# Alxkov/PSA-simulation-ODE-RK-MVP-Dispersion

Hardware: AMD Instinct MI355X
Metric: RK4 field-point updates/sec (sweep_pts x n_fields x n_zsteps / wall_s) (higher is better)
Workload: dtype f64

## Files before the change

psa-simulation-ode-rk-mvp-dispersion_amd/csrc/psa_rk4_kernel.inc.h:

```cpp
#pragma once
#include <type_traits>

#include "psa_internal.h"
#include "psa_rk4.h"

namespace psa {

__device__ __forceinline__ double fma_(double a, double b, double c) { return __builtin_fma(a, b, c); }
__device__ __forceinline__ float fma_(float a, float b, float c) { return __builtin_fmaf(a, b, c); }
typedef float f32x2 __attribute__((ext_vector_type(2)));
__device__ __forceinline__ f32x2 fma_(f32x2 a, f32x2 b, f32x2 c) { return __builtin_elementwise_fma(a, b, c); }

template <typename T> struct PairOf;
template <> struct PairOf<double> { typedef double type __attribute__((ext_vector_type(2))); };
template <> struct PairOf<float> { typedef float type __attribute__((ext_vector_type(2))); };

#ifndef PSA_TRAJ_F64_MOD
#define PSA_TRAJ_F64_MOD " nt"
#endif
__device__ __forceinline__ void store_pair_nt(const void *sbase, const unsigned voff, const PairOf<double>::type v) {
    asm volatile("global_store_dwordx4 %0, %1, %2" PSA_TRAJ_F64_MOD "\n\ts_nop 0\n\ts_nop 0" : : "v"(voff), "v"(v), "s"(sbase) : "memory");
}
__device__ __forceinline__ void store_pair_nt(const void *sbase, const unsigned voff, const PairOf<float>::type v) {
    asm volatile("global_store_dwordx2 %0, %1, %2 nt" : : "v"(voff), "v"(v), "s"(sbase) : "memory");
}
typedef float f32x4 __attribute__((ext_vector_type(4)));
__device__ __forceinline__ void store_quad_nt(const void *sbase, const unsigned voff, const f32x4 v) {
    asm volatile("global_store_dwordx4 %0, %1, %2 nt\n\ts_nop 0\n\ts_nop 0" : : "v"(voff), "v"(v), "s"(sbase) : "memory");
}

template <typename T> struct Phase;
template <> struct Phase<double> {
    static constexpr int RESYNC = 64;
    static __device__ __forceinline__ void eval(double ph, double &c, double &s) { sincos(ph, &s, &c); }
};
#ifndef PSA_F32_RESYNC
#define PSA_F32_RESYNC 16
#endif
template <> struct Phase<float> {
    static constexpr int RESYNC = PSA_F32_RESYNC;
    static __device__ __forceinline__ void eval(double ph, float &c, float &s) {
        const double r = ph - 6.283185307179586 * rint(ph * 0.15915494309189535);
        sincosf((float)r, &s, &c);
    }
};

template <typename T, int NW, bool FUSED, bool LOSS = true, bool CROSS = false, bool REALE = false>
__device__ __forceinline__ void yaman_stage(const T (&a)[2 * NW], const T (&base)[2 * NW],
                                            const T (&Er)[(NW - 2) / 2], const T (&Ei)[(NW - 2) / 2], const T g,
                                            const T tg, const T ha, T (&out)[2 * NW]) {
    static_assert(!REALE || (CROSS && NW == 4), "the real phase factor exists for the crosswise 4-wave stage");
    constexpr int NP = (NW - 2) / 2;
    T p[NW];
#pragma unroll
    for (int j = 0; j < NW; ++j) p[j] = fma_(a[2 * j], a[2 * j], a[2 * j + 1] * a[2 * j + 1]);
    T s = (p[0] + p[1]) + (p[2] + p[3]);
    if constexpr (NW == 6) s += (p[4] + p[5]);
    const T gs = tg * s;
    T gj[NW];
#pragma unroll
    for (int j = 0; j < NW; ++j) gj[j] = fma_(-g, p[j], gs);

    auto link = [&](const T gsig, const T v, const int c) -> T {
        if constexpr (LOSS) return fma_(gsig, v, FUSED ? fma_(ha, a[c], base[c]) : ha * a[c]);
        else return FUSED ? fma_(gsig, v, base[c]) : gsig * v;
    };

    const T x1 = a[0], y1 = a[1], x2 = a[2], y2 = a[3];
    if constexpr (CROSS && NW == 4) {
        const T x3 = a[4], y3 = a[5], x4 = a[6], y4 = a[7];
        const T b23r = fma_(x2, x3, y2 * y3), b23i = fma_(x2, y3, -(y2 * x3));
        const T b14r = fma_(x1, x4, y1 * y4), b14i = fma_(x1, y4, -(y1 * x4));
        const T h23r = REALE ? Er[0] * b23r : fma_(Er[0], b23r, -(Ei[0] * b23i));
        const T h23i = REALE ? Er[0] * b23i : fma_(Er[0], b23i, Ei[0] * b23r);
        const T h14r = REALE ? Er[0] * b14r : fma_(Er[0], b14r, -(Ei[0] * b14i));
        const T h14i = REALE ? Er[0] * b14i : fma_(Er[0], b14i, Ei[0] * b14r);
        out[0] = fma_(-y4, h23r, fma_(-x4, h23i, link(-gj[0], y1, 0)));
        out[1] = fma_(x4, h23r, fma_(-y4, h23i, link(gj[0], x1, 1)));
        out[2] = fma_(-y3, h14r, fma_(-x3, h14i, link(-gj[1], y2, 2)));
        out[3] = fma_(x3, h14r, fma_(-y3, h14i, link(gj[1], x2, 3)));
        out[4] = fma_(-y2, h14r, fma_(x2, h14i, link(-gj[2], y3, 4)));
        out[5] = fma_(x2, h14r, fma_(y2, h14i, link(gj[2], x3, 5)));
        out[6] = fma_(-y1, h23r, fma_(x1, h23i, link(-gj[3], y4, 6)));
        out[7] = fma_(x1, h23r, fma_(y1, h23i, link(gj[3], x4, 7)));
        return;
    }
    const T q12r = fma_(x1, x2, -(y1 * y2)), q12i = fma_(x1, y2, y1 * x2);

    T Fpr = T{}, Fpi = T{};
#pragma unroll
    for (int pr = 0; pr < NP; ++pr) {
        const int cs = 4 + 4 * pr;
        const T xs = a[cs], ys = a[cs + 1], xi = a[cs + 2], yi = a[cs + 3];
        const T qr = fma_(xs, xi, -(ys * yi)), qi = fma_(xs, yi, ys * xi);
        if (pr == 0) {
            Fpr = fma_(Er[pr], qr, -(Ei[pr] * qi));
            Fpi = fma_(Er[pr], qi, Ei[pr] * qr);
        } else {
            Fpr = fma_(Er[pr], qr, fma_(-Ei[pr], qi, Fpr));
            Fpi = fma_(Er[pr], qi, fma_(Ei[pr], qr, Fpi));
        }
        const T Fsr = fma_(Er[pr], q12r, Ei[pr] * q12i);
        const T Fsi = fma_(Er[pr], q12i, -(Ei[pr] * q12r));
        const T gS = gj[2 + 2 * pr], gI = gj[3 + 2 * pr];
        out[cs] = fma_(yi, Fsr, fma_(-xi, Fsi, link(-gS, ys, cs)));
        out[cs + 1] = fma_(xi, Fsr, fma_(yi, Fsi, link(gS, xs, cs + 1)));
        out[cs + 2] = fma_(ys, Fsr, fma_(-xs, Fsi, link(-gI, yi, cs + 2)));
        out[cs + 3] = fma_(xs, Fsr, fma_(ys, Fsi, link(gI, xi, cs + 3)));
    }
    out[0] = fma_(y2, Fpr, fma_(-x2, Fpi, link(-gj[0], y1, 0)));
    out[1] = fma_(x2, Fpr, fma_(y2, Fpi, link(gj[0], x1, 1)));
    out[2] = fma_(y1, Fpr, fma_(-x1, Fpi, link(-gj[1], y2, 2)));
    out[3] = fma_(x1, Fpr, fma_(y1, Fpi, link(gj[1], x2, 3)));
}

template <typename T, bool LOSS = true, bool FUSED = true, bool REALE = false>
__device__ __forceinline__ void yaman_stage_mirrored(const T (&a)[4], const T (&base)[4], const T Er, const T Ei, const T g,
                                                     const T sg, const T ha, T (&out)[4]) {
    const T x1 = a[0], y1 = a[1], xs = a[2], ys = a[3];
    const T p0 = fma_(x1, x1, y1 * y1), p2 = fma_(xs, xs, ys * ys);
    const T gs = sg * (p0 + p2);
    const T g1 = fma_(-g, p0, gs), g3 = fma_(-g, p2, gs);
    auto link = [&](const T gsig, const T v, const int c) -> T {
        if constexpr (LOSS) return fma_(gsig, v, FUSED ? fma_(ha, a[c], base[c]) : ha * a[c]);
        else return FUSED ? fma_(gsig, v, base[c]) : gsig * v;
    };
    const T br = fma_(x1, xs, y1 * ys), bi = fma_(x1, ys, -(y1 * xs));
    const T hr = REALE ? Er * br : fma_(Er, br, -(Ei * bi));
    const T hi = REALE ? Er * bi : fma_(Er, bi, Ei * br);
    out[0] = fma_(-ys, hr, fma_(-xs, hi, link(-g1, y1, 0)));
    out[1] = fma_(xs, hr, fma_(-ys, hi, link(g1, x1, 1)));
    out[2] = fma_(-y1, hr, fma_(x1, hi, link(-g3, ys, 2)));
    out[3] = fma_(x1, hr, fma_(y1, hi, link(g3, xs, 3)));
}

template <typename T, int NW, bool LOSS = true>
__device__ __forceinline__ void yaman_rhs(const T (&a)[2 * NW], const T (&Er)[(NW - 2) / 2],
                                          const T (&Ei)[(NW - 2) / 2], const T g, const T tg, const T ha,
                                          T (&k)[2 * NW]) {
    yaman_stage<T, NW, false, LOSS, true>(a, a, Er, Ei, g, tg, ha, k);
}

template <typename T>
__device__ __forceinline__ void rotate(T &Er, T &Ei, const T rc, const T rs) {
    const T nr = fma_(Er, rc, -(Ei * rs));
    const T ni = fma_(Er, rs, Ei * rc);
    Er = nr;
    Ei = ni;
}

template <typename T, int NC>
__device__ __forceinline__ bool any_nonfinite(const T (&y)[NC]) {
    T t = T(0);
#pragma unroll
    for (int c = 0; c < NC; ++c) t = fma_(y[c], T(0), t);
    return t != t;
}

#ifndef PSA_SWEEP_KERNEL_ATTR
#define PSA_SWEEP_KERNEL_ATTR
#endif
template <typename T, int NW, int CHECK, bool TRAJ, int BLOCK, bool LDS, bool LOSS, bool WSUM, bool MIRROR>
__device__ __forceinline__ void sweep_point(const SweepArgs<T> &A, const long long idx, T (&y)[MIRROR ? NW : 2 * NW]) {
    static_assert(!MIRROR || (sizeof(T) == 8 && NW == 4 && !LDS), "the mirrored body exists for the fused float64 4-wave step");
    constexpr int NC = 2 * NW;
    constexpr int NS = MIRROR ? NW : NC;
    constexpr int NWS = NS / 2;
    constexpr int SIG = MIRROR ? 2 : 4;
    constexpr int NP = (NW - 2) / 2;
    constexpr int RESYNC = Phase<T>::RESYNC;
    auto at = [](const int c) { return MIRROR ? (((c >> 2) << 1) | (c & 1)) : c; };
    const long long N = A.n_points;

    const T g = A.gamma[idx * A.gamma_stride];
    const T tg = g + g;
    const T ha = T(-0.5) * A.alpha[idx * A.alpha_stride];
    double dbd[NP];
    dbd[0] = (double)A.dbeta[idx];
    if constexpr (NP == 2) dbd[1] = (double)A.dbeta2[idx];

    const double hd = A.z_max / (double)A.n_steps;
    const T h = (T)hd, hh = (T)(0.5 * hd), h6 = (T)(hd / 6.0);
    const T g_d = hh * g, tg_d = hh * tg, ha_d = hh * ha;
    const T g_h = h * g, tg_h = h * tg, ha_h = h * ha;
    const T third = T(1.0 / 3.0);
    constexpr bool FUSE = (sizeof(T) == 8) && !LDS;
    const T e_amp = FUSE ? tg_d : tg;
    constexpr bool FRAME = FUSE && NW == 4;

    T rc[NP], rs[NP], Er[NP], Ei[NP];
#pragma unroll
    for (int p = 0; p < NP; ++p) {
        Phase<T>::eval(dbd[p] * (0.5 * hd), rc[p], rs[p]);
        Er[p] = e_amp;
        Ei[p] = T(0);
    }
    const T ec = e_amp * rc[0], es = e_amp * rs[0];
    auto frame_seed = [&](const int step, T &fc, T &fs) {
        Phase<T>::eval(dbd[0] * (0.5 * fma_((double)step, hd, 0.5 * hd)), fc, fs);
    };
    auto frame_at = [&](const int step, T &fc, T &fs) {
        const int k = step % RESYNC;
        frame_seed(step - k, fc, fs);
#pragma nounroll
        for (int q = 0; q < k; ++q) rotate(fc, fs, rc[0], rs[0]);
    };
    auto leave_frame = [&](const T (&b)[NS], const T fc, const T fs, T (&a)[NS]) {
        const T ce = T(-0.5) * fma_(fs, fs, fma_(fc, fc, T(-1)));
        const T nc = fma_(fc, ce, fc), ns = fma_(fs, ce, fs);
#pragma unroll
        for (int c = 0; c < SIG; ++c) a[c] = b[c];
#pragma unroll
        for (int c = SIG; c < NS; c += 2) {
            a[c] = fma_(b[c], nc, b[c + 1] * ns);
            a[c + 1] = fma_(b[c + 1], nc, -(b[c] * ns));
        }
    };
    T Fc = T(1), Fs = T(0);

    T pe = fma_(y[SIG], y[SIG], y[SIG + 1] * y[SIG + 1]);
    T pm = pe;
    long long bad = -1;
    T pwm[WSUM ? NWS : 1];
    if constexpr (WSUM) {
#pragma unroll
        for (int j = 0; j < NWS; ++j) pwm[j] = fma_(y[2 * j], y[2 * j], y[2 * j + 1] * y[2 * j + 1]);
    }
    auto store_a_end = [&](const T (&a)[NS]) {
#pragma unroll
        for (int c = 0; c < NC; ++c) A.a_end[(long long)c * N + idx] = a[at(c)];
        if constexpr (WSUM) {
#pragma unroll
            for (int j = 0; j < NW; ++j) {
                const T xr = y[at(2 * j)], xi = y[at(2 * j + 1)];
                A.p_wave_end[(long long)j * N + idx] = fma_(xr, xr, xi * xi);
            }
        }
    };

    const int se = A.save_every;
    const int n_rows = A.n_steps / se;
    const int n_run = (CHECK != CHECK_NONE) ? A.n_steps : n_rows * se;

    using Pair = typename PairOf<T>::type;
    const long long LD = A.traj_ld;
    const unsigned lane_off = (unsigned)idx * (unsigned)sizeof(Pair);
    auto store_traj_row_of = [&](const int r, const T (&a)[NS]) {
        const char *rowb = reinterpret_cast<const char *>(A.traj) + (long long)r * NW * LD * (long long)sizeof(Pair);
#pragma unroll
        for (int j = 0; j < NW; ++j)
            store_pair_nt(rowb + (long long)j * LD * (long long)sizeof(Pair), lane_off, Pair{a[at(2 * j)], a[at(2 * j + 1)]});
    };
    auto store_traj_row = [&](const int r) {
        if constexpr (FRAME) {
            T a[NS];
            leave_frame(y, Fc, Fs, a);
            store_traj_row_of(r, a);
        } else {
            store_traj_row_of(r, y);
        }
    };
    auto store_a_end_at = [&](const int step) {
        if constexpr (FRAME) {
            T a[NS], fc = Fc, fs = Fs;
            if constexpr (!TRAJ) frame_at(step, fc, fs);
            leave_frame(y, fc, fs, a);
            store_a_end(a);
        } else {
            store_a_end(y);
        }
    };
    if constexpr (TRAJ) store_traj_row_of(0, y);
    if (n_rows == 0) store_a_end(y);
    if constexpr (FRAME) {
        frame_seed(0, Fc, Fs);
#pragma unroll
        for (int c = SIG; c < NS; c += 2) rotate(y[c], y[c + 1], Fc, Fs);
    }

    __shared__ T sm_store[LDS ? 5 * NC * BLOCK : 1];
    volatile T *sm_y = sm_store + threadIdx.x;
    volatile T *sm_k = sm_store + NC * BLOCK + threadIdx.x;
    if constexpr (LDS) {
#pragma unroll
        for (int c = 0; c < NC; ++c) sm_y[c * BLOCK] = y[c];
    }
    auto rk4_step_lds = [&](const int step_index) {
        if constexpr (LDS) {
            T k[NC], ys[NC];
            const T coef[3] = {hh, hh, h};
#pragma unroll
            for (int c = 0; c < NC; ++c) ys[c] = sm_y[c * BLOCK];
#pragma unroll
            for (int st = 0; st < 4; ++st) {
                yaman_rhs<T, NW>(ys, Er, Ei, g, tg, ha, k);
#pragma unroll
                for (int c = 0; c < NC; ++c) sm_k[(st * NC + c) * BLOCK] = k[c];
                if (st == 0 || st == 2) {
#pragma unroll
                    for (int p = 0; p < NP; ++p) rotate(Er[p], Ei[p], rc[p], rs[p]);
                }
                if (st < 3) {
#pragma unroll
                    for (int c = 0; c < NC; ++c) ys[c] = fma_(coef[st], (T)sm_k[(st * NC + c) * BLOCK], (T)sm_y[c * BLOCK]);
                }
            }
#pragma unroll
            for (int c = 0; c < NC; ++c) {
                const T k1 = sm_k[(0 * NC + c) * BLOCK], k2 = sm_k[(1 * NC + c) * BLOCK];
                const T k3 = sm_k[(2 * NC + c) * BLOCK], k4 = sm_k[(3 * NC + c) * BLOCK];
                y[c] = fma_(h6, fma_(T(2), k3, fma_(T(2), k2, k1)) + k4, (T)sm_y[c * BLOCK]);
                sm_y[c * BLOCK] = y[c];
            }
            if constexpr (CHECK == CHECK_EXACT) {
                if (bad < 0 && any_nonfinite<T, NC>(y)) bad = step_index;
            }
        }
    };

    auto stage = [&](auto reale, const T (&a)[NS], const T (&base)[NS], const T (&er)[NP], const T (&ei)[NP], const T g_c,
                     const T tg_c, const T ha_c, T (&out)[NS]) {
        constexpr bool RE = decltype(reale)::value;
        if constexpr (MIRROR) yaman_stage_mirrored<T, LOSS, true, RE>(a, base, er[0], ei[0], g_c, tg_c + tg_c, ha_c, out);
        else yaman_stage<T, NW, true, LOSS, true, RE>(a, base, er, ei, g_c, tg_c, ha_c, out);
    };
    constexpr std::false_type cplx{};
    constexpr std::true_type real{};
    auto rk4_step_on = [&](T (&y)[NS], T (&Er)[NP], T (&Ei)[NP]) {
        T Y2[NS], Y3[NS], Y4[NS], t[NS], D[NS];
        if constexpr (FRAME) {
            const T c1[NP] = {ec}, s1[NP] = {-es}, s4[NP] = {es}, e1[NP] = {tg_d}, e2[NP] = {tg_h};
            stage(cplx, y, y, c1, s1, g_d, tg_d, ha_d, Y2);
            stage(real, Y2, y, e1, e1, g_d, tg_d, ha_d, Y3);
            stage(real, Y3, y, e2, e2, g_h, tg_h, ha_h, Y4);
#pragma unroll
            for (int c = 0; c < NS; ++c) t[c] = fma_(T(2), Y3[c], fma_(T(-4), y[c], Y2[c])) + Y4[c];
            stage(cplx, Y4, t, c1, s4, g_d, tg_d, ha_d, D);
#pragma unroll
            for (int c = 0; c < NS; ++c) y[c] = fma_(D[c], third, y[c]);
#pragma unroll
            for (int c = SIG; c < NS; c += 2) rotate(y[c], y[c + 1], rc[0], rs[0]);
            return;
        }
        stage(cplx, y, y, Er, Ei, g_d, tg_d, ha_d, Y2);
#pragma unroll
        for (int p = 0; p < NP; ++p) rotate(Er[p], Ei[p], rc[p], rs[p]);
        stage(cplx, Y2, y, Er, Ei, g_d, tg_d, ha_d, Y3);
        T E2r[NP], E2i[NP];
#pragma unroll
        for (int p = 0; p < NP; ++p) {
            E2r[p] = Er[p] + Er[p];
            E2i[p] = Ei[p] + Ei[p];
        }
        stage(cplx, Y3, y, E2r, E2i, g_h, tg_h, ha_h, Y4);
#pragma unroll
        for (int c = 0; c < NS; ++c) t[c] = fma_(T(2), Y3[c], fma_(T(-4), y[c], Y2[c])) + Y4[c];
#pragma unroll
        for (int p = 0; p < NP; ++p) rotate(Er[p], Ei[p], rc[p], rs[p]);
        stage(cplx, Y4, t, Er, Ei, g_d, tg_d, ha_d, D);
#pragma unroll
        for (int c = 0; c < NS; ++c) y[c] = fma_(D[c], third, y[c]);
    };
    auto rk4_step_reg = [&](const int) {
        rk4_step_on(y, Er, Ei);
        if constexpr (FRAME && TRAJ) rotate(Fc, Fs, rc[0], rs[0]);
    };

    T y_lo[NS];
#pragma unroll
    for (int c = 0; c < NS; ++c) y_lo[c] = T{};
    auto rk4_step_classic = [&](const int step_index) {
        if constexpr (!FUSE) {
            T k[NC], ys[NC], acc[NC];
            yaman_rhs<T, NW, LOSS>(y, Er, Ei, g, tg, ha, k);
#pragma unroll
            for (int c = 0; c < NC; ++c) {
                acc[c] = k[c];
                ys[c] = fma_(hh, k[c], y[c]);
            }
#pragma unroll
            for (int p = 0; p < NP; ++p) rotate(Er[p], Ei[p], rc[p], rs[p]);
            yaman_rhs<T, NW, LOSS>(ys, Er, Ei, g, tg, ha, k);
#pragma unroll
            for (int c = 0; c < NC; ++c) {
                acc[c] = fma_(T(2), k[c], acc[c]);
                ys[c] = fma_(hh, k[c], y[c]);
            }
            yaman_rhs<T, NW, LOSS>(ys, Er, Ei, g, tg, ha, k);
#pragma unroll
            for (int c = 0; c < NC; ++c) {
                acc[c] = fma_(T(2), k[c], acc[c]);
                ys[c] = fma_(h, k[c], y[c]);
            }
#pragma unroll
            for (int p = 0; p < NP; ++p) rotate(Er[p], Ei[p], rc[p], rs[p]);
            yaman_rhs<T, NW, LOSS>(ys, Er, Ei, g, tg, ha, k);
#pragma unroll
            for (int c = 0; c < NC; ++c) {
                const T inc = fma_(h6, acc[c] + k[c], y_lo[c]);
                const T sum = y[c] + inc;
                y_lo[c] = inc - (sum - y[c]);
                y[c] = sum;
            }
            if constexpr (CHECK == CHECK_EXACT) {
                if (bad < 0 && any_nonfinite<T, NC>(y)) bad = step_index;
            }
        }
    };
    auto rk4_step = [&](const int step_index) {
        if constexpr (FUSE) rk4_step_reg(step_index);
        else rk4_step_classic(step_index);
    };

    auto write_summary = [&]() {
        A.p_end[idx] = pe;
        A.p_max[idx] = pm;
        A.first_bad[idx] = bad;
        if constexpr (WSUM) {
#pragma unroll
            for (int j = 0; j < NW; ++j) A.p_wave_max[(long long)j * N + idx] = pwm[at(2 * j) / 2];
        }
    };
    auto seed_phase_on = [&](const int step, T (&Er)[NP], T (&Ei)[NP]) {
        const double z = (double)step * hd;
#pragma unroll
        for (int p = 0; p < NP; ++p) {
            T c, s;
            Phase<T>::eval(dbd[p] * z, c, s);
            Er[p] = e_amp * c;
            Ei[p] = e_amp * s;
        }
    };
    auto seed_phase = [&](const int step) { seed_phase_on(step, Er, Ei); };

    constexpr bool REPLAY = FUSE && CHECK == CHECK_EXACT;
    T y_chk[REPLAY ? NS : 1], Er_chk[REPLAY && !FRAME ? NP : 1], Ei_chk[REPLAY && !FRAME ? NP : 1];
    int i_chk = 0;
    auto checkpoint = [&](const int step) {
        if constexpr (REPLAY) {
#pragma unroll
            for (int c = 0; c < NS; ++c) y_chk[c] = y[c];
            if constexpr (!FRAME) {
#pragma unroll
                for (int p = 0; p < NP; ++p) {
                    Er_chk[p] = Er[p];
                    Ei_chk[p] = Ei[p];
                }
            }
            i_chk = step;
        }
    };
    auto exact_test = [&](const int i_now) {
        if constexpr (REPLAY) {
            const bool newly_bad = bad < 0 && any_nonfinite<T, NS>(y);
            if (__builtin_amdgcn_ballot_w64(newly_bad) != 0) {
                T yy[NS], er[NP], ei[NP];
#pragma unroll
                for (int c = 0; c < NS; ++c) yy[c] = y_chk[c];
#pragma unroll
                for (int p = 0; p < NP; ++p) {
                    er[p] = FRAME ? T(0) : Er_chk[FRAME ? 0 : p];
                    ei[p] = FRAME ? T(0) : Ei_chk[FRAME ? 0 : p];
                }
                int ii = i_chk;
                while (ii < i_now) {
                    if constexpr (!FRAME) {
                        if (ii % RESYNC == 0) seed_phase_on(ii, er, ei);
                    }
                    const int to_seed = FRAME ? i_now - ii : RESYNC - ii % RESYNC;
                    const int e = (i_now - ii > to_seed) ? ii + to_seed : i_now;
#pragma nounroll
                    for (int st = ii; st < e; ++st) {
                        rk4_step_on(yy, er, ei);
                        if (bad < 0 && any_nonfinite<T, NS>(yy)) bad = st;
                    }
                    ii = e;
                }
            }
            checkpoint(i_now);
        }
    };

    if constexpr (TRAJ && !LDS) {
        if (se == 1) {
            auto save_row = [&](const int r) {
                pe = fma_(y[SIG], y[SIG], y[SIG + 1] * y[SIG + 1]);
                pm = pe > pm ? pe : pm;
                if constexpr (CHECK == CHECK_BLOCK || (CHECK == CHECK_EXACT && FUSE)) {
                    if (bad < 0 && any_nonfinite<T, NS>(y)) bad = r - 1;
                }
                store_traj_row(r);
            };
            int i = 0;
            while (i < n_run) {
                if constexpr (!FRAME) seed_phase(i);
                const int end = (n_run - i > RESYNC) ? i + RESYNC : n_run;
                for (; i + 2 <= end; i += 2) {
                    rk4_step(i);
                    save_row(i + 1);
                    rk4_step(i + 1);
                    if constexpr (FRAME) {
                        if ((i + 2) % RESYNC == 0) frame_seed(i + 2, Fc, Fs);
                    }
                    save_row(i + 2);
                }
                if (i < end) {
                    rk4_step(i);
                    save_row(i + 1);
                    ++i;
                }
            }
            if (pe != pe) pm = pe;
            if constexpr (FRAME) {
                T a[NS];
                leave_frame(y, Fc, Fs, a);
#pragma unroll
                for (int c = 0; c < NC; ++c) A.a_end[(long long)c * N + idx] = a[at(c)];
            } else {
#pragma unroll
                for (int c = 0; c < NC; ++c) A.a_end[(long long)c * N + idx] = y[at(c)];
            }
            write_summary();
            return;
        }
    }

    int i = 0;
    int row = 0;
    checkpoint(0);
    int next_save = (n_rows > 0) ? se : 0x7fffffff;
    int next_seed = !FRAME ? 0 : ((TRAJ && n_run >= RESYNC) ? RESYNC : 0x7fffffff);
    while (i < n_run) {
        if constexpr (!FRAME) {
            if (i == next_seed) {
                seed_phase(i);
                next_seed = (n_run - i > RESYNC) ? i + RESYNC : 0x7fffffff;
            }
        }
        int end = n_run < next_seed ? n_run : next_seed;
        end = end < next_save ? end : next_save;
        const int m = end - i;
        int j = 0;
        if constexpr (LDS) {
            for (; j < m; ++j) rk4_step_lds(i + j);
        } else {
            for (; j + 2 <= m; j += 2) {
                rk4_step(i + j);
                rk4_step(i + j + 1);
            }
            if (j < m) rk4_step(i + j);
        }
        i = end;
        if constexpr (FRAME && TRAJ) {
            if (i == next_seed) {
                frame_seed(i, Fc, Fs);
                next_seed = (n_run - i >= RESYNC) ? i + RESYNC : 0x7fffffff;
            }
        }
        if (i == next_save) {
            ++row;
            pe = fma_(y[SIG], y[SIG], y[SIG + 1] * y[SIG + 1]);
            pm = (pe > pm || pe != pe) ? pe : pm;
            if constexpr (WSUM) {
#pragma unroll
                for (int j = 0; j < NWS; ++j) {
                    const T pj = fma_(y[2 * j], y[2 * j], y[2 * j + 1] * y[2 * j + 1]);
                    pwm[j] = (pj > pwm[j] || pj != pj) ? pj : pwm[j];
                }
            }
            if constexpr (CHECK == CHECK_BLOCK) {
                if (bad < 0 && any_nonfinite<T, NS>(y)) bad = i - 1;
            }
            exact_test(i);
            if constexpr (TRAJ) store_traj_row(row);
            if (row == n_rows) {
                store_a_end_at(i);
                next_save = 0x7fffffff;
            } else {
                next_save += se;
            }
        }
    }
    if constexpr (CHECK == CHECK_BLOCK) {
        if (bad < 0 && n_run > 0 && any_nonfinite<T, NS>(y)) bad = n_run - 1;
    }
    if (n_run > i_chk) exact_test(n_run);
    write_summary();
}

__device__ __forceinline__ bool wave_starts_mirrored(const double (&y)[8]) {
    bool same = true;
#pragma unroll
    for (int c = 0; c < 8; c += 4) {
        same = same && __builtin_bit_cast(long long, y[c]) == __builtin_bit_cast(long long, y[c + 2]) &&
               __builtin_bit_cast(long long, y[c + 1]) == __builtin_bit_cast(long long, y[c + 3]);
    }
    const bool objects = !same || any_nonfinite<double, 8>(y);
    return __builtin_amdgcn_ballot_w64(objects) == 0;
}

template <typename T, int NW, int CHECK, bool TRAJ, int BLOCK, bool LDS = false, bool LOSS = true, bool WSUM = false>
__global__ void __launch_bounds__(BLOCK) PSA_SWEEP_KERNEL_ATTR rk4_sweep_kernel(const SweepArgs<T> A) {
    static_assert(!WSUM || (!TRAJ && !LDS), "the per-wave summary exists for the register layout without trajectory");
    constexpr int NC = 2 * NW;
    const long long idx = (long long)blockIdx.x * BLOCK + threadIdx.x;
    if (idx >= A.n_points) return;

    T y[NC];
#pragma unroll
    for (int c = 0; c < NC; ++c) y[c] = A.a0[(long long)c * A.a0_ld + idx * A.a0_stride];
    if constexpr (sizeof(T) == 8 && NW == 4 && !LDS) {
        if (wave_starts_mirrored(y)) {
            long long idx_m = idx;
            asm volatile("" : "+v"(idx_m));
            T ym[NW];
#pragma unroll
            for (int c = 0; c < NW; ++c) ym[c] = A.a0[(long long)(c < 2 ? c : c + 2) * A.a0_ld + idx_m * A.a0_stride];
            sweep_point<T, NW, CHECK, TRAJ, BLOCK, LDS, LOSS, WSUM, true>(A, idx_m, ym);
            return;
        }
    }
    sweep_point<T, NW, CHECK, TRAJ, BLOCK, LDS, LOSS, WSUM, false>(A, idx, y);
}

template <typename T> struct OneLane {
    static long long lanes(long long n_points) { return n_points; }
    template <int NW, int CHECK, bool TRAJ, int BLOCK, bool LDS, bool LOSS, bool WSUM>
    static constexpr auto kernel() {
        if constexpr ((WSUM && (TRAJ || LDS || BLOCK != 256)) || (LDS && (BLOCK != 64 || !LOSS))) return nullptr;
        else return rk4_sweep_kernel<T, NW, CHECK, TRAJ, BLOCK, LDS, LOSS, WSUM>;
    }
};

struct Pick {
    int n_waves, check, block;
    bool traj, lds, lossless, wsum;
};

template <typename T>
static Pick pick_one_lane(int n_waves, uint32_t flags, const SweepArgs<T> &a) {
    Pick p;
    p.n_waves = n_waves;
    p.check = !(flags & PSA_OPT_CHECK_NAN) ? CHECK_NONE : ((flags & PSA_OPT_EXACT_STEP) ? CHECK_EXACT : CHECK_BLOCK);
    p.traj = a.traj != nullptr;
    p.wsum = a.p_wave_end != nullptr;
    p.lds = (flags & PSA_OPT_LDS_STAGING) != 0;
    p.lossless = (flags & PSA_OPT_LOSSLESS) && !p.lds;
    p.block = (p.lds || (flags & PSA_OPT_BLOCK64)) ? 64 : 256;
    return p;
}

template <int V, int... Vs, typename F>
static hipError_t with_int(int v, F &&f) {
    if constexpr (sizeof...(Vs) == 0) return f(std::integral_constant<int, V>{});
    else return v == V ? f(std::integral_constant<int, V>{}) : with_int<Vs...>(v, f);
}
template <typename F>
static hipError_t with_bool(bool b, F &&f) { return b ? f(std::true_type{}) : f(std::false_type{}); }

template <typename Family, typename T>
static hipError_t launch_family(hipStream_t s, const Pick &p, const SweepArgs<T> &a) {
    if (a.n_points == 0) return hipSuccess;
    const dim3 grid((unsigned)((Family::lanes(a.n_points) + p.block - 1) / p.block)), block(p.block);
    return with_int<4, 6>(p.n_waves, [&](auto nw) {
    return with_int<CHECK_NONE, CHECK_BLOCK, CHECK_EXACT>(p.check, [&](auto check) {
    return with_int<64, 256>(p.block, [&](auto blk) {
    return with_bool(p.traj, [&](auto traj) {
    return with_bool(p.lds, [&](auto lds) {
    return with_bool(p.lossless, [&](auto lossless) {
    return with_bool(p.wsum, [&](auto wsum) {
        constexpr auto k = Family::template kernel<nw, check, traj, blk, lds, !lossless, wsum>();
        if constexpr (std::is_null_pointer_v<std::remove_const_t<decltype(k)>>) {
            return hipErrorInvalidDeviceFunction;
        } else {
            void *args[] = {const_cast<SweepArgs<T> *>(&a)};
            (void)hipLaunchKernel(reinterpret_cast<const void *>(k), grid, block, args, 0, s);
            return hipGetLastError();
        }
    }); }); }); }); }); }); });
}

}
```

Baseline: 910.2 billion.

## Add specialized unrolled row loop for frame-mode runs without trajectory output

New measurement: 928.1 billion (median of 6 runs). +2.0%, better.

```diff
diff --git a/psa-simulation-ode-rk-mvp-dispersion_amd/csrc/psa_rk4_kernel.inc.h b/psa-simulation-ode-rk-mvp-dispersion_amd/csrc/psa_rk4_kernel.inc.h
--- a/psa-simulation-ode-rk-mvp-dispersion_amd/csrc/psa_rk4_kernel.inc.h
+++ b/psa-simulation-ode-rk-mvp-dispersion_amd/csrc/psa_rk4_kernel.inc.h
@@ -525,6 +525,80 @@
         }
     }
 
+#ifndef PSA_ROW_TRIP
+#define PSA_ROW_TRIP 4
+#endif
+    if constexpr (FRAME && !TRAJ) {
+        static_assert(PSA_ROW_TRIP == 4 || PSA_ROW_TRIP == 2, "the row loop runs 4 or 2 steps per trip");
+        auto write_powers = [&]() {
+            A.p_end[idx] = pe;
+            A.p_max[idx] = pm;
+            if constexpr (WSUM) {
+#pragma unroll
+                for (int j = 0; j < NW; ++j) A.p_wave_max[(long long)j * N + idx] = pwm[at(2 * j) / 2];
+            }
+        };
+        const int tail = n_run - n_rows * se;
+        const int rows_per_test = se < 64 ? 64 / se : 1;
+        auto span_of = [&](const int rows) { return (REPLAY && rows > rows_per_test) ? rows_per_test : rows; };
+        int left = n_rows > 0 ? n_rows : -1;
+        int m = left < 0 ? tail : se;
+        int trips = m / PSA_ROW_TRIP;
+        int span = left < 0 ? 1 : span_of(left);
+        [[maybe_unused]] int i_row = 0;
+        checkpoint(0);
+        if (left < 0) write_powers();
+        if (m > 0) {
+            for (int until = span;;) {
+                if (m & 1) rk4_step_reg(0);
+                if constexpr (PSA_ROW_TRIP == 4) {
+                    if (m & 2) {
+                        rk4_step_reg(0);
+                        rk4_step_reg(0);
+                    }
+                }
+                for (int q = trips; q > 0; --q) {
+                    rk4_step_reg(0);
+                    rk4_step_reg(0);
+                    if constexpr (PSA_ROW_TRIP == 4) {
+                        rk4_step_reg(0);
+                        rk4_step_reg(0);
+                    }
+                }
+                pe = fma_(y[SIG], y[SIG], y[SIG + 1] * y[SIG + 1]);
+                pm = (pe > pm || pe != pe) ? pe : pm;
+                if constexpr (WSUM) {
+#pragma unroll
+                    for (int j = 0; j < NWS; ++j) {
+                        const T pj = fma_(y[2 * j], y[2 * j], y[2 * j + 1] * y[2 * j + 1]);
+                        pwm[j] = (pj > pwm[j] || pj != pj) ? pj : pwm[j];
+                    }
+                }
+                if constexpr (CHECK == CHECK_BLOCK) {
+                    i_row += m;
+                    if (bad < 0 && any_nonfinite<T, NS>(y)) bad = i_row - 1;
+                }
+                if (--until != 0) continue;
+                if (left > 0) left -= span;
+                exact_test(left < 0 ? n_run : (n_rows - left) * se);
+                if (left < 0) break;
+                if (left > 0) {
+                    until = span = span_of(left);
+                    continue;
+                }
+                store_a_end_at(n_rows * se);
+                write_powers();
+                if (tail == 0) break;
+                left = -1;
+                m = tail;
+                trips = m / PSA_ROW_TRIP;
+                until = 1;
+            }
+        }
+        A.first_bad[idx] = bad;
+        return;
+    }
+
     int i = 0;
     int row = 0;
     checkpoint(0);
```
